# physimals/fabber_core

Hardware: AMD Instinct MI355X
Metric: voxels/sec to VB convergence (higher is better)
Workload: dtype f64; 1 GPU; BASELINE configs[2]: bi-exponential (examples biexp), white noise, 100 timepoints, max-iterations 50; voxels_per_gpu=1000000, total_voxels=1000000, params=4, need_f=False, parallelism=voxel-shard x1, input_dtype=f32, bad_voxels=55

## Files before the change

fabber_core_amd/csrc/vb_lane_kernel.h:

```cpp
#pragma once

#include "vb_math.h"
#include "vb_models.h"

namespace fvb
{
template <int P>
constexpr int lane_waves()
{
#ifdef FVB_LANE_WAVES_PER_SIMD
    return FVB_LANE_WAVES_PER_SIMD;
#else
    return P <= 2 ? 3 : (P >= 7 ? 1 : 2);
#endif
}
template <int P>
constexpr int lane_prefetch_depth()
{
#ifdef FVB_PREFETCH_DEPTH
    return FVB_PREFETCH_DEPTH;
#else
    return P <= 2 ? 2 : 4;
#endif
}
// ... 175 lines not shown
        if constexpr (ACC)
        {
            if (precise)
                sweep.step_acc(ma, t, tp, tp2, tp3, rden, g, J);
            else
                sweep.eval_jac(ma, t, tp, tp2, tp3, rden, g, J);
        }
        else
            sweep.eval_jac(ma, t, tp, tp2, tp3, rden, g, J);
        if (phi_index)
        {
#pragma unroll
            for (int i = 0; i < P; i++)
                bad_jac |= !is_finite(J[i]);
        }
        if (phi_index)
            bad_offset |= !is_finite(g);
        else
            g_total += g;
        const bool unmasked = phi_index ? (phi_index[t] != 255) : true;
        if (unmasked)
        {
            const double r = y_cur - g;
#pragma unroll
            for (int i = 0; i < P; i++)
            {
#pragma unroll
                for (int j = 0; j <= i; j++)
                    mo.A[tri(i, j)] += J[i] * J[j];
                mo.u[i] += J[i] * r;
            }
            mo.s += r * r;
        }
    };
    FVB_FOR_EACH_TIMEPOINT(lane_prefetch_depth<P>(), ka, v, V, T, step)
    if (!phi_index)
    {
        bad_offset = !is_finite(g_total);
#pragma unroll
        for (int i = 0; i < P; i++)
            bad_jac |= !is_finite(mo.A[tri(i, i)]);
    }
    return bad_offset ? FVB_BAD_OFFSET : (bad_jac ? FVB_BAD_JACOBIAN : FVB_OK);
}

enum
{
    FEED_TILES_F32 = 0,
    FEED_TILES_F64 = 1,
    FEED_STRIDED = 2
};

template <int FEED>
struct FeedTraits
{
    typedef float raw;
};
template <>
struct FeedTraits<FEED_TILES_F64>
{
    typedef double raw;
};

template <typename RAW>
struct Tile
{
    static constexpr int G = 16 / (int)sizeof(RAW);
    typedef RAW vec __attribute__((ext_vector_type(16 / sizeof(RAW))));
    static FVB_HD size_t groups(int T)
    {
        return (size_t)((T + G - 1) / G);
    }
    static FVB_HD size_t block_elems(int T)
    {
        return groups(T) * 64 * G;
    }
    static FVB_HD size_t bytes(int V, int T)
    {
        return (size_t)((V + 63) / 64) * block_elems(T) * sizeof(RAW);
    }
};

template <typename RAW>
__global__ __launch_bounds__(256) void retile_series(const RAW *__restrict__ data, RAW *__restrict__ tiles, int V, int T)
{
    typedef Tile<RAW> TL;
    const int v = blockIdx.x * 256 + threadIdx.x;
    if (v >= V)
        return;
    const int n_groups = (int)TL::groups(T);
    typename TL::vec *dst = (typename TL::vec *)(tiles + (size_t)(v >> 6) * TL::block_elems(T)) + (v & 63);
    const RAW *src = data + v;
    for (int g = 0; g < n_groups; g++)
    {
        typename TL::vec q;
#pragma unroll
        for (int j = 0; j < TL::G; j++)
        {
            const int t = g * TL::G + j;
            q[j] = (t < T) ? src[(size_t)t * V] : RAW(0);
        }
        dst[(size_t)g * 64] = q;
    }
}

template <typename RAW, class Body>
__device__ __forceinline__ void for_each_timepoint_tiled(const RAW *lane_tile, int T, Body body)
{
    typedef Tile<RAW> TL;
    constexpr int TRIP = 8;
    constexpr int NL = TRIP / TL::G;
    const int n_trips = T / TRIP;
    if (n_trips > 0)
    {
        const typename TL::vec *p = (const typename TL::vec *)lane_tile;
        typename TL::vec qa[NL], qb[NL];
        auto fetch = [&](typename TL::vec(&q)[NL], int trip) {
#pragma unroll
            for (int l = 0; l < NL; l++)
                q[l] = p[(size_t)(trip * NL + l) * 64];
        };
        auto process = [&](const typename TL::vec(&q)[NL], int t0) {
#pragma unroll
            for (int j = 0; j < TRIP; j++)
                body(t0 + j, (double)q[j / TL::G][j % TL::G]);
        };
        fetch(qa, 0);
        int k = 0;
        for (; k + 2 <= n_trips; k += 2)
        {
            fetch(qb, k + 1);
            process(qa, k * TRIP);
            fetch(qa, (k + 2 < n_trips) ? k + 2 : n_trips - 1);
            process(qb, (k + 1) * TRIP);
        }
        if (k < n_trips)
            process(qa, k * TRIP);
    }
#pragma nounroll
    for (int t = n_trips * TRIP; t < T; t++)
        body(t, (double)lane_tile[(size_t)(t / TL::G) * 64 * TL::G + (t % TL::G)]);
}

template <class Model, int P, typename RAW>
__device__ __forceinline__ int recentre_tiles(const KernelArgs &ka, const ModelArgs &ma, const RAW *lane_tile,
    const double (&centre)[P], Moments<P> &mo, bool precise, double *sweep_park = nullptr)
{
    typedef Tile<RAW> TL;
    constexpr int PT = P * (P + 1) / 2;
    constexpr int TRIP = 8;
    constexpr int NL = TRIP / TL::G;
    static_assert(FVB_EXP_RESYNC == 1 || FVB_EXP_RESYNC == 2 || FVB_EXP_RESYNC == 4 || FVB_EXP_RESYNC == 8,
        "the resync period must divide the trip length");
    const int T = ka.cfg.n_times;
    double tp[P], tp2[P], tp3[P], rden[P];
#pragma unroll
    for (int i = 0; i < P; i++)
    {
        const int tr = ka.cfg.transform[i];
        double delta = centre[i] * 1e-5;
        if (delta < 0)
            delta = -delta;
        if (delta < 1e-10)
            delta = 1e-10;
        const double c2 = centre[i] + delta;
        const double c3 = centre[i] - delta;
        tp[i] = to_model(tr, centre[i]);
        tp2[i] = to_model(tr, c2);
        tp3[i] = to_model(tr, c3);
        rden[i] = 1.0 / (c2 - c3);
        mo.ml[i] = centre[i];
    }
    if (sweep_park)
    {
        double *q = sweep_park + (threadIdx.x & 63);
#pragma unroll
        for (int i = 0; i < P; i++)
        {
            q[(0 * P + i) * 64] = tp[i];
            q[(1 * P + i) * 64] = tp2[i];
            q[(2 * P + i) * 64] = tp3[i];
            q[(3 * P + i) * 64] = rden[i];
        }
    }
#pragma unroll
    for (int i = 0; i < PT; i++)
        mo.A[i] = 0;
#pragma unroll
    for (int i = 0; i < P; i++)
        mo.u[i] = 0;
    mo.s = 0;
    mo.precise = precise;
    typename Model::Sweep sweep;
    sweep.init(ma, tp, tp2, tp3);
    sweep.set_precise(false);
    double g_total = 0;
    auto accumulate = [&](double y_cur, double g, const double(&J)[P]) {
        g_total += g;
        const double r = y_cur - g;
#pragma unroll
        for (int i = 0; i < P; i++)
        {
#pragma unroll
            for (int j = 0; j <= i; j++)
                mo.A[tri(i, j)] += J[i] * J[j];
            mo.u[i] += J[i] * r;
        }
        mo.s += r * r;
    };
    int t = 0;
    const int n_trips = precise ? 0 : T / TRIP;
    if (n_trips > 0)
    {
        const typename TL::vec *p = (const typename TL::vec *)lane_tile;
        typename TL::vec qa[NL], qb[NL];
        auto fetch = [&](typename TL::vec(&q)[NL], int trip) {
#pragma unroll
            for (int l = 0; l < NL; l++)
                q[l] = p[(size_t)(trip * NL + l) * 64];
        };
        auto process = [&](const typename TL::vec(&q)[NL], int t0) {
#pragma unroll
            for (int j = 0; j < TRIP; j++)
            {
                double g, J[P];
                if (j % FVB_EXP_RESYNC == 0)
                    sweep.template step_fast<true>(ma, t0 + j, tp, tp2, tp3, rden, g, J);
                else
                    sweep.template step_fast<false>(ma, t0 + j, tp, tp2, tp3, rden, g, J);
                accumulate((double)q[j / TL::G][j % TL::G], g, J);
            }
        };
        fetch(qa, 0);
        int k = 0;
        for (; k + 2 <= n_trips; k += 2)
        {
            fetch(qb, k + 1);
            process(qa, k * TRIP);
            fetch(qa, (k + 2 < n_trips) ? k + 2 : n_trips - 1);
            process(qb, (k + 1) * TRIP);
        }
        if (k < n_trips)
            process(qa, k * TRIP);
        t = n_trips * TRIP;
    }
#pragma nounroll
    for (; t < T; t++)
    {
        const double y_cur = (double)lane_tile[(size_t)(t / TL::G) * 64 * TL::G + (t % TL::G)];
        double g, J[P];
        sweep.step_any(ma, t, tp, tp2, tp3, rden, g, J, precise);
        accumulate(y_cur, g, J);
    }
    bool bad_jac = false;
#pragma unroll
    for (int i = 0; i < P; i++)
        bad_jac |= !is_finite(mo.A[tri(i, i)]);
    return !is_finite(g_total) ? FVB_BAD_OFFSET : (bad_jac ? FVB_BAD_JACOBIAN : FVB_OK);
}

template <int P, bool NEEDF>
__device__ __forceinline__ bool apply_priors(const KernelArgs &ka, int v, int it, VoxelState<P> &st, double &Fprior)
{
    bool ok = true;
    bool any_ard = false;
#pragma unroll
    for (int k = 0; k < P; k++)
        any_ard |= (ka.cfg.prior_type[k] == FVB_PRIOR_ARD);
    if (any_ard)
        ok = ensure_cov<P>(st);
#pragma unroll
    for (int k = 0; k < P; k++)
    {
        const int type = ka.cfg.prior_type[k];
        double fk = 0;
        double pm_k, pprec_k;
        if (type == FVB_PRIOR_ARD)
        {
            const double post_mean = st.m[k];
            const double post_cov = st.Sig[tri(k, k)];
            const double new_cov = post_mean * post_mean + post_cov;
            pprec_k = 1.0 / ((it == 0) ? ka.cfg.prior_var[k] : new_cov);
            pm_k = ka.cfg.prior_mean[k];
            if (NEEDF)
            {
                const double bb = 2 / new_cov;
                fk = -1.5 * (log(bb) + digamma(0.5)) - 0.5 - gammaln(0.5) - 0.5 * log(bb);
            }
        }
        else if (type == FVB_PRIOR_IMAGE)
        {
            pm_k = ka.cfg.image_prior[k][v];
            pprec_k = ka.cfg.prior_prec[k];
        }
        else
        {
            pm_k = ka.cfg.prior_mean[k];
            pprec_k = ka.cfg.prior_prec[k];
        }
        st.pm[k] = pm_k;
        st.pprec[k] = pprec_k;
        Fprior = fk;
    }
    return ok;
}

template <int P>
__device__ __forceinline__ double theta_rhs_base(double phibar, const Moments<P> &mo, int i)
{
    double aml = 0;
#pragma unroll
    for (int j = 0; j < P; j++)
        aml = __builtin_fma(mo.A[tri(i, j)], mo.ml[j], aml);
    return phibar * (mo.u[i] + aml);
}
__device__ __forceinline__ double theta_rhs(double base, double prior_prec, double prior_mean)
{
    return __builtin_fma(prior_prec, prior_mean, base);
}
template <int P>
__device__ __forceinline__ double theta_mean(const double *Sig, const double (&rhs)[P], int i)
{
    double s = 0;
#pragma unroll
    for (int j = 0; j < P; j++)
        s = __builtin_fma(Sig[tri(i, j)], rhs[j], s);
    return s;
}

template <int P>
__device__ __forceinline__ bool update_theta(VoxelState<P> &st, const Moments<P> &mo, double alpha)
{
    constexpr int PT = P * (P + 1) / 2;
    const double phibar = st.b * st.c;
#pragma unroll
    for (int i = 0; i < P; i++)
#pragma unroll
        for (int j = 0; j <= i; j++)
            st.Lam[tri(i, j)] = phibar * mo.A[tri(i, j)] + ((i == j) ? st.pprec[i] : 0.0);
    st.precValid = true;
    st.covValid = false;
    if (alpha <= 0.0)
    {
        double rhs[P];
#pragma unroll
        for (int i = 0; i < P; i++)
            rhs[i] = theta_rhs(theta_rhs_base<P>(phibar, mo, i), st.pprec[i], st.pm[i]);
        if (!ensure_cov<P>(st))
            return false;
#pragma unroll
        for (int i = 0; i < P; i++)
            st.m[i] = theta_mean<P>(st.Sig, rhs, i);
    }
    else
    {
        double Delta[P], Mx[PT], Mi[PT];
#pragma unroll
        for (int i = 0; i < P; i++)
            Delta[i] = phibar * mo.u[i] + st.pprec[i] * st.pm[i] - st.pprec[i] * mo.ml[i];
#pragma unroll
        for (int i = 0; i < PT; i++)
            Mx[i] = st.Lam[i];
#pragma unroll
        for (int i = 0; i < P; i++)
            Mx[tri(i, i)] += alpha * st.Lam[tri(i, i)];
        double la;
        int sg;
        if (ldl_inverse<P>(Mx, Mi, la, sg))
        {
#pragma unroll
            for (int i = 0; i < P; i++)
            {
                double s = 0;
#pragma unroll
                for (int j = 0; j < P; j++)
                    s += Mi[tri(i, j)] * Delta[j];
                st.m[i] = mo.ml[i] + s;
            }
        }
    }
    return true;
}

template <int P>
__device__ __forceinline__ double trace_SA(const VoxelState<P> &st, const Moments<P> &mo)
{
    double tr = 0;
#pragma unroll
    for (int i = 0; i < P; i++)
#pragma unroll
        for (int j = 0; j < P; j++)
            tr += st.Sig[tri(i, j)] * mo.A[tri(i, j)];
    return tr;
}

template <int P>
__device__ __forceinline__ void residual_terms(
    const VoxelState<P> &st, const Moments<P> &mo, double tol, double &kk, double &trSA, bool &lost)
{
    double d[P];
#pragma unroll
    for (int i = 0; i < P; i++)
        d[i] = st.m[i] - mo.ml[i];
    double du = 0, dAd = 0;
    trSA = 0;
// ... 532 lines not shown
    {
        lg = gammaln(c);
        dg = digamma(c);
    }
    const double noise_terms = free_energy_noise_terms(ka, b, c, lg, dg, fk.prior_const);
    const double prior_logdet = (fk.prior_is_const && priors_applied) ? fk.prior_logdet : prior_log_determinant<P>(st);
    double F = theta_terms + noise_terms + data_terms + prior_logdet;
    finite = is_finite(F);
    return F + Fprior;
}

template <int P>
__device__ __forceinline__ bool free_energy_would_be_finite(const VoxelState<P> &st, double theta_terms, double data_terms)
{
    bool ok = is_finite(theta_terms + data_terms) && st.b > 0 && st.c > 0 && is_finite(st.b * st.c) && is_finite(st.c);
#pragma unroll
    for (int i = 0; i < P; i++)
        ok = ok && is_finite(st.pprec[i]) && st.pprec[i] != 0;
    return ok;
}

template <int P>
__device__ __forceinline__ void save_state(const KernelArgs &ka, int v, const VoxelState<P> &st)
{
    constexpr int PT = P * (P + 1) / 2;
    const size_t V = (size_t)ka.cfg.n_voxels;
    double *p = ka.save + v;
    int r = 0;
#pragma unroll
    for (int i = 0; i < P; i++)
        p[(size_t)(r++) * V] = st.m[i];
#pragma unroll
    for (int i = 0; i < PT; i++)
        p[(size_t)(r++) * V] = st.Lam[i];
#pragma unroll
    for (int i = 0; i < PT; i++)
        p[(size_t)(r++) * V] = st.Sig[i];
#pragma unroll
    for (int i = 0; i < P; i++)
        p[(size_t)(r++) * V] = st.pm[i];
#pragma unroll
    for (int i = 0; i < P; i++)
        p[(size_t)(r++) * V] = st.pprec[i];
    p[(size_t)(r++) * V] = st.b;
    p[(size_t)(r++) * V] = st.c;
    p[(size_t)(r++) * V] = (st.precValid ? 1.0 : 0.0) + (st.covValid ? 2.0 : 0.0) + 4.0 * 0;
}

template <int P>
__device__ __forceinline__ void restore_state(const KernelArgs &ka, int v, VoxelState<P> &st)
{
    constexpr int PT = P * (P + 1) / 2;
    const size_t V = (size_t)ka.cfg.n_voxels;
    const double *p = ka.save + v;
    int r = 0;
#pragma unroll
    for (int i = 0; i < P; i++)
        st.m[i] = p[(size_t)(r++) * V];
#pragma unroll
    for (int i = 0; i < PT; i++)
        st.Lam[i] = p[(size_t)(r++) * V];
#pragma unroll
    for (int i = 0; i < PT; i++)
        st.Sig[i] = p[(size_t)(r++) * V];
#pragma unroll
    for (int i = 0; i < P; i++)
        st.pm[i] = p[(size_t)(r++) * V];
#pragma unroll
    for (int i = 0; i < P; i++)
        st.pprec[i] = p[(size_t)(r++) * V];
    st.b = p[(size_t)(r++) * V];
    st.c = p[(size_t)(r++) * V];
    const int flags = (int)p[(size_t)(r++) * V];
    if (flags & 1)
    {
        st.precValid = true;
        st.covValid = false;
    }
    else
    {
        st.precValid = false;
        st.covValid = true;
    }
}

template <class Model, int P, bool NEEDF, int FEED, bool WATCH = NEEDF>
__global__ __launch_bounds__(64, lane_waves<P>()) void vb_lane_kernel(const KernelArgs ka)
{
    constexpr int PT = P * (P + 1) / 2;
    typedef typename FeedTraits<FEED>::raw RAW;
    const int v_lane = blockIdx.x * 64 + threadIdx.x;
    const int v = (v_lane < ka.cfg.n_voxels) ? v_lane : ka.cfg.n_voxels - 1;
    const int T = ka.cfg.n_times;
    const size_t V = (size_t)ka.cfg.n_voxels;

    ModelArgs ma;
    ma.iopt0 = ka.cfg.model_iopt[0];
    ma.dopt0 = ka.cfg.model_dopt[0];
    ma.design = ka.cfg.design;
    const RAW *wave_tile = (FEED == FEED_STRIDED) ? nullptr : (const RAW *)ka.tiles + (size_t)blockIdx.x * Tile<RAW>::block_elems(T);
    const RAW *lane_tile = (FEED == FEED_STRIDED) ? nullptr : wave_tile + (size_t)(v & 63) * Tile<RAW>::G;

    VoxelState<P> st;
    Moments<P> mo;
    int status = FVB_OK;
    __shared__ double park_lds[ParkPlan<P, NEEDF>::ROWS * 64];
    __shared__ double rescue_row[64];
    constexpr bool SWEEP_PARKED = (FEED != FEED_STRIDED) && SweepPark<P, NEEDF>::FITS;
    __shared__ double sweep_lds[SWEEP_PARKED ? SweepPark<P, NEEDF>::ROWS * 64 : 1];
    double *park = park_lds + threadIdx.x;
    double *sweep_park = SWEEP_PARKED ? sweep_lds : nullptr;

    if (ka.cfg.init_mvn)
    {
        constexpr int n = P + 1;
        constexpr int nCov = n * (n + 1) / 2;
        const double *src = ka.cfg.init_mvn + v;
#pragma unroll
        for (int i = 0; i < PT; i++)
            st.Sig[i] = src[(size_t)i * V];
#pragma unroll
        for (int i = 0; i < P; i++)
            st.m[i] = src[(size_t)(nCov + i) * V];
        const double nm = src[(size_t)(nCov + P) * V];
        const double nv = src[(size_t)tri(P, P) * V];
        st.b = nv / nm;
        st.c = nm / st.b;
    }
    else
    {
#pragma unroll
        for (int i = 0; i < PT; i++)
            st.Sig[i] = 0;
#pragma unroll
        for (int i = 0; i < P; i++)
        {
            st.m[i] = (ka.cfg.prior_type[i] == FVB_PRIOR_IMAGE) ? ka.cfg.image_prior[i][v] : ka.cfg.post_mean[i];
            st.Sig[tri(i, i)] = ka.cfg.post_var[i];
        }
        if (Model::needs_data_max)
        {
            double data_max;
            if (FEED == FEED_STRIDED)
            {
                data_max = load_data(ka, v);
                for (int t = 1; t < T; t++)
                {
                    const double y = load_data(ka, (size_t)t * V + v);
                    data_max = (y > data_max) ? y : data_max;
                }
            }
            else
            {
                constexpr int G = Tile<RAW>::G;
                data_max = (double)lane_tile[0];
#pragma nounroll
                for (int t = 1; t < T; t++)
                {
                    const double y = (double)lane_tile[(size_t)(t / G) * 64 * G + (t % G)];
                    data_max = (y > data_max) ? y : data_max;
                }
            }
            Model::init_posterior(ma, data_max, st.m);
        }
#pragma unroll
        for (int i = 0; i < P; i++)
        {
            const int tr = ka.cfg.transform[i];
            st.m[i] = to_fabber(tr, st.m[i]);
            st.Sig[tri(i, i)] = to_fabber_var(tr, st.Sig[tri(i, i)]);
        }
        st.b = ka.cfg.noise_post_b[0];
        st.c = ka.cfg.noise_post_c[0];
    }
    st.covValid = true;
    st.precValid = false;
    st.logdetLam = 0;
#pragma unroll
    for (int i = 0; i < P; i++)
    {
        st.pm[i] = 0;
        st.pprec[i] = 1;
    }

    double F = 1234.5678;
    double Fprior = 0;
    int it = 0;
    int hist_len = 0;
    bool setup_failed = false;

    ConvState conv;
    conv_init(conv, ka.cfg.convergence, ka.cfg.max_iterations, ka.cfg.max_trials, ka.cfg.min_fchange);
    conv_reset(conv);
    const bool use_save = WATCH && (ka.save != nullptr);
    enum
    {
        FIRST,
        ITERATING,
        REVERTED
    };
    int phase = FIRST;
    int n_lin = 0;
    bool logdet_valid = false;

    enum
    {
        LINEARISE,
        PRIORS,
        THETA,
        NOISE
    };
    int stage = LINEARISE;
    double kk = 0, trSA = 0;
    FreeEnergyConsts<P> fk;
    if (NEEDF)
        fk.init(ka);
    bool pending = false, priors_applied = false;
    double pending_part = 0, pending_b = 0, pending_c = 0;
#define FVB_VOXEL_FAILS(CODE, B, C)                                                                          \
    {                                                                                                        \
        status = (CODE);                                                                                     \
        pending_b = (B);                                                                                     \
        pending_c = (C);                                                                                     \
        break;                                                                                               \
    }
    for (;;)
    {
        bool want_f = NEEDF;
        double f_kk, f_tr;
        double b_before = 0, c_before = 0;
        if (stage == LINEARISE)
        {
            park_state<P, NEEDF>(park, st);
            if (FEED == FEED_STRIDED)
                status = recentre<Model, P>(ka, ma, v, st.m, mo, n_lin < ka.precise_passes);
            else
                status = recentre_tiles<Model, P, RAW>(ka, ma, lane_tile, st.m, mo, n_lin < ka.precise_passes, sweep_park);
            n_lin = (phase == REVERTED) ? n_lin : n_lin + 1;
            unpark_state<P, NEEDF>(park, st);
            if (status != FVB_OK)
            {
                setup_failed = (phase == FIRST);
                FVB_VOXEL_FAILS(status, st.b, st.c)
            }
            if (phase == FIRST)
            {
                if (use_save)
                    save_posterior<P>(ka, v, st, logdet_valid);
                want_f = false;
            }
        }
        else if (stage == PRIORS)
        {
            if (use_save && conv_need_save(conv))
                save_posterior<P>(ka, v, st, logdet_valid);
            if (!apply_priors<P, NEEDF>(ka, v, it, st, Fprior))
                FVB_VOXEL_FAILS(FVB_BAD_RESULT, st.b, st.c)
            priors_applied = true;
        }
        else if (stage == THETA)
        {
            if (!update_theta<P>(st, mo, WATCH ? conv_lm_alpha(conv) : 0.0) || !ensure_cov<P>(st))
                FVB_VOXEL_FAILS(FVB_BAD_RESULT, st.b, st.c)
            st.precValid = false;
            logdet_valid = true;
            if (FEED == FEED_STRIDED)
                residual_and_trace<Model, P, NEEDF>(ka, ma, v, st, mo, kk, trSA, park, rescue_row);
            else
                residual_and_trace_adaptive<Model, P, NEEDF, RAW, SWEEP_PARKED>(ka, ma, v, st, mo, kk, trSA, park, rescue_row, wave_tile, sweep_park);
        }
        else
        {
            b_before = st.b;
            c_before = st.c;
            update_noise<P>(ka, st, kk, trSA);
        }
        if (want_f)
        {
            if (stage == LINEARISE || stage == PRIORS)
            {
                if (!ensure_cov<P>(st))
                    FVB_VOXEL_FAILS(FVB_BAD_RESULT, st.b, st.c)
                f_kk = mo.s;
                f_tr = trace_SA<P>(st, mo);
            }
            else
            {
                f_kk = kk;
                f_tr = trSA;
            }
            double theta_terms, data_terms;
            if (!free_energy_partial<P>(ka, st, f_kk, f_tr, logdet_valid, theta_terms, data_terms))
                FVB_VOXEL_FAILS(FVB_BAD_RESULT, st.b, st.c)
            if (stage == LINEARISE)
            {
                bool fin = true;
                const double Fn = free_energy_full<P>(ka, fk, st, st.b, st.c, priors_applied && phase != REVERTED, theta_terms, data_terms, Fprior, fin);
                if (!fin)
                    FVB_VOXEL_FAILS(FVB_BAD_FREE_ENERGY, st.b, st.c)
                F = Fn;
                pending = false;
            }
            else
            {
                if (!free_energy_would_be_finite<P>(st, theta_terms, data_terms))
                {
                    const bool noise_stage = (stage == NOISE);
                    FVB_VOXEL_FAILS(FVB_BAD_FREE_ENERGY, noise_stage ? b_before : st.b, noise_stage ? c_before : st.c)
                }
                pending_part = theta_terms + data_terms;
                pending = true;
            }
        }
// ... 76 lines not shown
```

fabber_core_amd/csrc/vb_models.h:

```cpp
#pragma once

#include "vb_math.h"

#ifdef FVB_STRICT_MODELS
#define FVB_MODEL_FP _Pragma("clang fp contract(off)")
#else
#define FVB_MODEL_FP _Pragma("clang fp contract(fast)")
#endif

namespace fvb
{
struct ModelArgs
{
    int32_t iopt0;
    double dopt0;
    const double *design;
    const double *lin;
    int32_t lin_T;
    const double *exp_table;
    const double *consts;
    int32_t n_consts;
    int32_t model;
};

template <class Model, int P>
struct PointwiseSweep
{
    FVB_HD void init(const ModelArgs &, const double (&)[P], const double (&)[P], const double (&)[P])
    {
    }
    FVB_HD void set_precise(bool)
    {
    }
    FVB_HD void eval(const ModelArgs &ma, int t, const double (&tp)[P], const double (&tp2)[P], const double (&tp3)[P],
        double &g, double (&f2)[P], double (&f3)[P])
    {
        FVB_MODEL_FP
        g = Model::eval(ma, t, tp);
#pragma unroll
        for (int i = 0; i < P; i++)
        {
            double q[P];
#pragma unroll
            for (int j = 0; j < P; j++)
                q[j] = tp[j];
            q[i] = tp2[i];
            f2[i] = Model::eval(ma, t, q);
            q[i] = tp3[i];
            f3[i] = Model::eval(ma, t, q);
        }
    }
    FVB_HD void eval_jac(const ModelArgs &ma, int t, const double (&tp)[P], const double (&tp2)[P], const double (&tp3)[P],
        const double (&rden)[P], double &g, double (&J)[P])
    {
        FVB_MODEL_FP
        double f2[P], f3[P];
        eval(ma, t, tp, tp2, tp3, g, f2, f3);
#pragma unroll
        for (int i = 0; i < P; i++)
            J[i] = (f2[i] - f3[i]) * rden[i];
    }
    template <bool EXACT>
    FVB_HD void step_fast(const ModelArgs &ma, int t, const double (&tp)[P], const double (&tp2)[P],
        const double (&tp3)[P], const double (&rden)[P], double &g, double (&J)[P])
    {
        eval_jac(ma, t, tp, tp2, tp3, rden, g, J);
    }
    FVB_HD void step_any(const ModelArgs &ma, int t, const double (&tp)[P], const double (&tp2)[P],
        const double (&tp3)[P], const double (&rden)[P], double &g, double (&J)[P], bool)
    {
        eval_jac(ma, t, tp, tp2, tp3, rden, g, J);
    }
};

template <class Model, int P>
struct LinearInParameterSweep
{
    double d2[P], d3[P];
    bool precise;
    FVB_HD void init(const ModelArgs &, const double (&tp)[P], const double (&tp2)[P], const double (&tp3)[P])
    {
        precise = false;
#pragma unroll
        for (int i = 0; i < P; i++)
        {
            d2[i] = tp2[i] - tp[i];
            d3[i] = tp3[i] - tp[i];
        }
    }
    FVB_HD void set_precise(bool p)
    {
        precise = p;
    }
    FVB_HD void eval(const ModelArgs &ma, int t, const double (&tp)[P], const double (&tp2)[P], const double (&tp3)[P],
        double &g, double (&f2)[P], double (&f3)[P])
    {
        FVB_MODEL_FP
        if (precise)
        {
            PointwiseSweep<Model, P> pw;
            pw.eval(ma, t, tp, tp2, tp3, g, f2, f3);
            return;
        }
        g = Model::eval(ma, t, tp);
#pragma unroll
        for (int i = 0; i < P; i++)
        {
            const double b = Model::basis(ma, t, i);
            f2[i] = g + b * d2[i];
            f3[i] = g + b * d3[i];
        }
    }
    FVB_HD void eval_jac(const ModelArgs &ma, int t, const double (&tp)[P], const double (&tp2)[P], const double (&tp3)[P],
        const double (&rden)[P], double &g, double (&J)[P])
    {
        FVB_MODEL_FP
        if (precise)
        {
            PointwiseSweep<Model, P> pw;
            pw.eval_jac(ma, t, tp, tp2, tp3, rden, g, J);
            return;
        }
        g = Model::eval(ma, t, tp);
#pragma unroll
        for (int i = 0; i < P; i++)
            J[i] = Model::basis(ma, t, i) * ((tp2[i] - tp3[i]) * rden[i]);
    }
    template <bool EXACT>
    FVB_HD void step_fast(const ModelArgs &ma, int t, const double (&tp)[P], const double (&tp2)[P],
        const double (&tp3)[P], const double (&rden)[P], double &g, double (&J)[P])
    {
        FVB_MODEL_FP
        g = Model::eval(ma, t, tp);
#pragma unroll
        for (int i = 0; i < P; i++)
            J[i] = Model::basis(ma, t, i) * ((tp2[i] - tp3[i]) * rden[i]);
    }
    FVB_HD void step_any(const ModelArgs &ma, int t, const double (&tp)[P], const double (&tp2)[P],
        const double (&tp3)[P], const double (&rden)[P], double &g, double (&J)[P], bool prec)
    {
        precise = prec;
        eval_jac(ma, t, tp, tp2, tp3, rden, g, J);
    }
};

template <int P>
struct PolyModel
{
    static constexpr bool host_evaluated = false;
    static constexpr int model_id = FVB_MODEL_POLY;
    typedef LinearInParameterSweep<PolyModel<P>, P> Sweep;
    static FVB_HD double basis(const ModelArgs &, int t, int n)
    {
        int pw = 1;
        for (int k = 0; k < n; k++)
            pw *= t + 1;
        return (double)pw;
    }
    static FVB_HD double eval(const ModelArgs &, int t, const double (&p)[P])
    {
        FVB_MODEL_FP
        const int i = t + 1;
        double res = 0;
        int pw = 1;
#pragma unroll
        for (int n = 0; n < P; n++)
        {
            res += p[n] * pw;
            pw *= i;
        }
        return res;
    }
    static FVB_HD void init_posterior(const ModelArgs &, double, double (&)[P])
    {
    }
    static constexpr bool needs_data_max = false;
};

template <int P>
struct LinearModel
{
    static constexpr bool host_evaluated = false;
    static constexpr int model_id = FVB_MODEL_LINEAR;
    typedef LinearInParameterSweep<LinearModel<P>, P> Sweep;
    static FVB_HD double basis(const ModelArgs &a, int t, int n)
    {
        return a.design[(size_t)t * P + n];
    }
    static FVB_HD double eval(const ModelArgs &a, int t, const double (&p)[P])
    {
        FVB_MODEL_FP
        const double *row = a.design + (size_t)t * P;
        double s = 0;
#pragma unroll
        for (int j = 0; j < P; j++)
            s += row[j] * (p[j] - 0.0);
        return s + 0.0;
    }
    static FVB_HD void init_posterior(const ModelArgs &, double, double (&)[P])
    {
    }
    static constexpr bool needs_data_max = false;
};

template <int P>
struct ExpModel
{
    static constexpr bool host_evaluated = false;
    static_assert(P % 2 == 0, "exp model has 2 parameters per exponential");
    static constexpr int model_id = FVB_MODEL_EXP;
    static FVB_HD double eval(const ModelArgs &a, int t, const double (&p)[P])
    {
        FVB_MODEL_FP
        const double tt = double(t) * a.dopt0;
        double res = 0;
#pragma unroll
        for (int i = 0; i < P / 2; i++)
        {
            double val = p[2 * i] * exp(-p[2 * i + 1] * tt);
            res += val;
        }
        return res;
    }
    static FVB_HD void init_posterior(const ModelArgs &, double data_max, double (&means)[P])
    {
#pragma unroll
        for (int i = 0; i < P / 2; i++)
            means[2 * i] = data_max / (P / 2 + i);
    }
    static constexpr bool needs_data_max = true;

#ifndef FVB_EXP_RESYNC
#define FVB_EXP_RESYNC 8
#endif
    struct Sweep
    {
        static constexpr int N = P / 2;
        double e0[N], e2[N], e3[N], s0[N], s2[N], s3[N];
        bool precise;
        FVB_HD void init(const ModelArgs &a, const double (&tp)[P], const double (&tp2)[P], const double (&tp3)[P])
        {
            FVB_MODEL_FP
            precise = false;
            if (FVB_EXP_RESYNC > 1)
            {
#pragma unroll
                for (int i = 0; i < N; i++)
                {
                    s0[i] = exp(-tp[2 * i + 1] * a.dopt0);
                    s2[i] = exp(-tp2[2 * i + 1] * a.dopt0);
                    s3[i] = exp(-tp3[2 * i + 1] * a.dopt0);
                }
            }
        }
        FVB_HD void set_precise(bool p)
        {
            precise = p;
        }
        FVB_HD void advance(const ModelArgs &a, int t, const double (&tp)[P], const double (&tp2)[P], const double (&tp3)[P])
        {
            FVB_MODEL_FP
            if (FVB_EXP_RESYNC <= 1 || precise || (t % FVB_EXP_RESYNC) == 0)
            {
                const double tt = double(t) * a.dopt0;
#pragma unroll
                for (int i = 0; i < N; i++)
                {
                    e0[i] = exp(-tp[2 * i + 1] * tt);
                    e2[i] = exp(-tp2[2 * i + 1] * tt);
                    e3[i] = exp(-tp3[2 * i + 1] * tt);
                }
            }
            else
            {
#pragma unroll
                for (int i = 0; i < N; i++)
                {
                    e0[i] *= s0[i];
                    e2[i] *= s2[i];
                    e3[i] *= s3[i];
                }
            }
        }
        FVB_HD void eval(const ModelArgs &a, int t, const double (&tp)[P], const double (&tp2)[P], const double (&tp3)[P],
            double &g, double (&f2)[P], double (&f3)[P])
        {
            FVB_MODEL_FP
            advance(a, t, tp, tp2, tp3);
            combine(tp, tp2, tp3, g, f2, f3);
        }
        FVB_HD void resync(const ModelArgs &a, int t, const double (&tp)[P], const double (&tp2)[P], const double (&tp3)[P])
        {
            FVB_MODEL_FP
            const double tt = double(t) * a.dopt0;
#pragma unroll
            for (int i = 0; i < N; i++)
            {
                e0[i] = exp(-tp[2 * i + 1] * tt);
                e2[i] = exp(-tp2[2 * i + 1] * tt);
                e3[i] = exp(-tp3[2 * i + 1] * tt);
            }
        }
        FVB_HD void resync_acc(const ModelArgs &a, int t, const double (&tp)[P], const double (&tp2)[P], const double (&tp3)[P])
        {
            FVB_MODEL_FP
            const double tt = double(t) * a.dopt0;
#pragma unroll
            for (int i = 0; i < N; i++)
            {
                e0[i] = exp_acc(-tp[2 * i + 1] * tt, a.exp_table);
                e2[i] = exp_acc(-tp2[2 * i + 1] * tt, a.exp_table);
                e3[i] = exp_acc(-tp3[2 * i + 1] * tt, a.exp_table);
            }
        }
        FVB_HD void multiply()
        {
            FVB_MODEL_FP
#pragma unroll
            for (int i = 0; i < N; i++)
            {
                e0[i] *= s0[i];
                e2[i] *= s2[i];
                e3[i] *= s3[i];
            }
        }
        FVB_HD void combine(const double (&tp)[P], const double (&tp2)[P], const double (&tp3)[P], double &g,
            double (&f2)[P], double (&f3)[P])
        {
            FVB_MODEL_FP
            double val[N];
#pragma unroll
            for (int j = 0; j < N; j++)
                val[j] = tp[2 * j] * e0[j];
            double res = val[0];
#pragma unroll
            for (int j = 1; j < N; j++)
                res += val[j];
            g = res;
#pragma unroll
            for (int i = 0; i < N; i++)
            {
                double a2 = (i == 0) ? tp2[0] * e0[0] : val[0];
                double a3 = (i == 0) ? tp3[0] * e0[0] : val[0];
                double r2 = (i == 0) ? tp[0] * e2[0] : val[0];
                double r3 = (i == 0) ? tp[0] * e3[0] : val[0];
#pragma unroll
                for (int j = 1; j < N; j++)
                {
                    a2 += (j == i) ? tp2[2 * i] * e0[i] : val[j];
                    a3 += (j == i) ? tp3[2 * i] * e0[i] : val[j];
                    r2 += (j == i) ? tp[2 * i] * e2[i] : val[j];
                    r3 += (j == i) ? tp[2 * i] * e3[i] : val[j];
                }
                f2[2 * i] = a2;
                f3[2 * i] = a3;
                f2[2 * i + 1] = r2;
                f3[2 * i + 1] = r3;
            }
        }
        FVB_HD void eval_jac(const ModelArgs &a, int t, const double (&tp)[P], const double (&tp2)[P], const double (&tp3)[P],
            const double (&rden)[P], double &g, double (&J)[P])
        {
            FVB_MODEL_FP
            double f2[P], f3[P];
            eval(a, t, tp, tp2, tp3, g, f2, f3);
#pragma unroll
            for (int i = 0; i < P; i++)
                J[i] = (f2[i] - f3[i]) * rden[i];
        }
        template <bool EXACT>
        FVB_HD void step_fast(const ModelArgs &a, int t, const double (&tp)[P], const double (&tp2)[P],
            const double (&tp3)[P], const double (&rden)[P], double &g, double (&J)[P])
        {
            FVB_MODEL_FP
            if (EXACT || FVB_EXP_RESYNC <= 1)
                resync(a, t, tp, tp2, tp3);
            else
                multiply();
            double f2[P], f3[P];
            combine(tp, tp2, tp3, g, f2, f3);
#pragma unroll
            for (int i = 0; i < P; i++)
                J[i] = (f2[i] - f3[i]) * rden[i];
        }
        FVB_HD void step_acc(const ModelArgs &a, int t, const double (&tp)[P], const double (&tp2)[P], const double (&tp3)[P],
            const double (&rden)[P], double &g, double (&J)[P])
        {
            FVB_MODEL_FP
            resync_acc(a, t, tp, tp2, tp3);
            double f2[P], f3[P];
            combine(tp, tp2, tp3, g, f2, f3);
#pragma unroll
            for (int i = 0; i < P; i++)
                J[i] = (f2[i] - f3[i]) * rden[i];
        }
        FVB_HD void step_any(const ModelArgs &a, int t, const double (&tp)[P], const double (&tp2)[P],
            const double (&tp3)[P], const double (&rden)[P], double &g, double (&J)[P], bool prec)
        {
            FVB_MODEL_FP
            if (FVB_EXP_RESYNC <= 1 || prec || (t % FVB_EXP_RESYNC) == 0)
                resync(a, t, tp, tp2, tp3);
            else
                multiply();
            double f2[P], f3[P];
            combine(tp, tp2, tp3, g, f2, f3);
#pragma unroll
            for (int i = 0; i < P; i++)
                J[i] = (f2[i] - f3[i]) * rden[i];
        }
    };
};

template <int P>
struct HostLinModel
{
    static constexpr bool host_evaluated = true;
    static constexpr int model_id = FVB_MODEL_HOSTJAC;
    static constexpr bool needs_data_max = false;
    static FVB_HD void init_posterior(const ModelArgs &, double, double (&)[P])
    {
    }
    static FVB_HD double eval(const ModelArgs &, int, const double (&)[P])
    {
        return __builtin_nan("");
    }
    struct Sweep
    {
        const double *g_row, *j_rows;
        FVB_HD void init(const ModelArgs &a, const double (&)[P], const double (&)[P], const double (&)[P])
        {
            g_row = a.lin;
            j_rows = a.lin + a.lin_T;
        }
        FVB_HD void set_precise(bool)
        {
        }
        FVB_HD void eval_jac(const ModelArgs &, int t, const double (&)[P], const double (&)[P], const double (&)[P],
            const double (&)[P], double &g, double (&J)[P])
        {
            g = g_row[t];
#pragma unroll
            for (int i = 0; i < P; i++)
                J[i] = j_rows[(size_t)t * P + i];
        }
    };
};

FVB_HD double eval_model_runtime(int model, const ModelArgs &a, int P, int t, const double *p)
{
    FVB_MODEL_FP
    switch (model)
    {
    case FVB_MODEL_POLY:
    {
        const int i = t + 1;
        double res = 0;
        int pw = 1;
        for (int n = 0; n < P; n++)
        {
            res += p[n] * pw;
            pw *= i;
        }
        return res;
    }
    case FVB_MODEL_LINEAR:
    {
        const double *row = a.design + (size_t)t * P;
        double s = 0;
        for (int j = 0; j < P; j++)
            s += row[j] * (p[j] - 0.0);
        return s + 0.0;
    }
    case FVB_MODEL_EXP:
    {
        const double tt = double(t) * a.dopt0;
        double res = 0;
        for (int i = 0; i < P / 2; i++)
            res += p[2 * i] * exp(-p[2 * i + 1] * tt);
        return res;
    }
    default:
        return NAN;
    }
}

}
```

Measured before the change: 74.65 million voxels/s.

## Run precise and remainder sweeps by prefetched trips and vectorise data-max scan

Restructures recentre_tiles so the tile prefetch is hoisted before the setup math. Precise sweeps and the tail remainder for multi-exponential models now go through the trip-based prefetched loop instead of a scalar per-timepoint loop. Adds an FMA-fused sum variant in combine for two-component models, and rewrites the data_max initial scan to use vector tile loads with a lookahead buffer. This aims to hide load latency and cut per-element index arithmetic, at the cost of more code paths and slightly different floating-point rounding from the fused sums.

```diff
diff --git a/fabber_core_amd/csrc/vb_lane_kernel.h b/fabber_core_amd/csrc/vb_lane_kernel.h
--- a/fabber_core_amd/csrc/vb_lane_kernel.h
+++ b/fabber_core_amd/csrc/vb_lane_kernel.h
@@ -351,7 +351,23 @@
     constexpr int NL = TRIP / TL::G;
     static_assert(FVB_EXP_RESYNC == 1 || FVB_EXP_RESYNC == 2 || FVB_EXP_RESYNC == 4 || FVB_EXP_RESYNC == 8,
         "the resync period must divide the trip length");
+    typedef typename Model::Sweep Sweep;
+    constexpr bool BY_TRIPS = Sweep::pointwise_by_trips;
     const int T = ka.cfg.n_times;
+    const int n_trips = (!BY_TRIPS && precise) ? 0 : T / TRIP;
+    const int rem = T - n_trips * TRIP;
+    const int last_group = (int)TL::groups(T) - 1;
+    const typename TL::vec *p = (const typename TL::vec *)lane_tile;
+    typename TL::vec qa[NL], qb[NL];
+    auto fetch = [&](typename TL::vec(&q)[NL], int trip) {
+#pragma unroll
+        for (int l = 0; l < NL; l++)
+        {
+            const int g = trip * NL + l;
+            q[l] = p[(size_t)(g < last_group ? g : last_group) * 64];
+        }
+    };
+    fetch(qa, 0);
     double tp[P], tp2[P], tp3[P], rden[P];
 #pragma unroll
     for (int i = 0; i < P; i++)
@@ -390,7 +406,7 @@
         mo.u[i] = 0;
     mo.s = 0;
     mo.precise = precise;
-    typename Model::Sweep sweep;
+    Sweep sweep;
     sweep.init(ma, tp, tp2, tp3);
     sweep.set_precise(false);
     double g_total = 0;
@@ -407,49 +423,128 @@
         }
         mo.s += r * r;
     };
-    int t = 0;
-    const int n_trips = precise ? 0 : T / TRIP;
-    if (n_trips > 0)
-    {
-        const typename TL::vec *p = (const typename TL::vec *)lane_tile;
-        typename TL::vec qa[NL], qb[NL];
-        auto fetch = [&](typename TL::vec(&q)[NL], int trip) {
-#pragma unroll
-            for (int l = 0; l < NL; l++)
-                q[l] = p[(size_t)(trip * NL + l) * 64];
-        };
-        auto process = [&](const typename TL::vec(&q)[NL], int t0) {
-#pragma unroll
-            for (int j = 0; j < TRIP; j++)
-            {
-                double g, J[P];
-                if (j % FVB_EXP_RESYNC == 0)
-                    sweep.template step_fast<true>(ma, t0 + j, tp, tp2, tp3, rden, g, J);
+    auto step = [&](bool exact, bool pointwise, bool fuse_last, int t, double &g, double(&J)[P]) {
+        if constexpr (Sweep::states_fusion)
+        {
+            if (pointwise)
+            {
+                if (fuse_last)
+                    sweep.template step_pointwise<2>(ma, t, tp, tp2, tp3, rden, g, J);
                 else
-                    sweep.template step_fast<false>(ma, t0 + j, tp, tp2, tp3, rden, g, J);
-                accumulate((double)q[j / TL::G][j % TL::G], g, J);
-            }
-        };
-        fetch(qa, 0);
+                    sweep.template step_pointwise<1>(ma, t, tp, tp2, tp3, rden, g, J);
+            }
+            else if (exact)
+            {
+                if (fuse_last)
+                    sweep.template step_fast<true, 2>(ma, t, tp, tp2, tp3, rden, g, J);
+                else
+                    sweep.template step_fast<true, 1>(ma, t, tp, tp2, tp3, rden, g, J);
+            }
+            else
+            {
+                if (fuse_last)
+                    sweep.template step_fast<false, 2>(ma, t, tp, tp2, tp3, rden, g, J);
+                else
+                    sweep.template step_fast<false, 1>(ma, t, tp, tp2, tp3, rden, g, J);
+            }
+        }
+        else
+        {
+            if (pointwise)
+                sweep.step_pointwise(ma, t, tp, tp2, tp3, rden, g, J);
+            else if (exact)
+                sweep.template step_fast<true>(ma, t, tp, tp2, tp3, rden, g, J);
+            else
+                sweep.template step_fast<false>(ma, t, tp, tp2, tp3, rden, g, J);
+        }
+    };
+    auto process = [&](const typename TL::vec(&q)[NL], int t0, bool second_of_pair) {
+#pragma unroll
+        for (int j = 0; j < TRIP; j++)
+        {
+            double g, J[P];
+            step(j % FVB_EXP_RESYNC == 0, false, j >= TRIP - (second_of_pair ? 2 : 1), t0 + j, g, J);
+            accumulate((double)q[j / TL::G][j % TL::G], g, J);
+        }
+    };
+    auto process_pointwise = [&](const typename TL::vec(&q)[NL], int t0) {
+#pragma unroll
+        for (int j = 0; j < TRIP; j++)
+        {
+            double g, J[P];
+            step(true, true, true, t0 + j, g, J);
+            accumulate((double)q[j / TL::G][j % TL::G], g, J);
+        }
+    };
+    auto next_set = [&]() {
+#pragma unroll
+        for (int l = 0; l < NL; l++)
+            qa[l] = qb[l];
+    };
+    if (precise)
+    {
+#pragma nounroll
+        for (int k = 0; k < n_trips; k++)
+        {
+            fetch(qb, k + 1);
+            process_pointwise(qa, k * TRIP);
+            next_set();
+        }
+    }
+    else
+    {
         int k = 0;
         for (; k + 2 <= n_trips; k += 2)
         {
             fetch(qb, k + 1);
-            process(qa, k * TRIP);
-            fetch(qa, (k + 2 < n_trips) ? k + 2 : n_trips - 1);
-            process(qb, (k + 1) * TRIP);
+            process(qa, k * TRIP, false);
+            fetch(qa, k + 2);
+            process(qb, (k + 1) * TRIP, true);
         }
         if (k < n_trips)
-            process(qa, k * TRIP);
-        t = n_trips * TRIP;
-    }
+        {
+            fetch(qb, k + 1);
+            process(qa, k * TRIP, false);
+            next_set();
+        }
+    }
+    int t_rem = n_trips * TRIP;
+    if constexpr (!BY_TRIPS)
+    {
 #pragma nounroll
-    for (; t < T; t++)
-    {
-        const double y_cur = (double)lane_tile[(size_t)(t / TL::G) * 64 * TL::G + (t % TL::G)];
-        double g, J[P];
-        sweep.step_any(ma, t, tp, tp2, tp3, rden, g, J, precise);
-        accumulate(y_cur, g, J);
+        for (int t = t_rem; t < T; t++)
+        {
+            const double y_cur = (double)lane_tile[(size_t)(t / TL::G) * 64 * TL::G + (t % TL::G)];
+            double g, J[P];
+            sweep.step_any(ma, t, tp, tp2, tp3, rden, g, J, precise);
+            accumulate(y_cur, g, J);
+        }
+    }
+    if constexpr (BY_TRIPS)
+        asm volatile("" : "+s"(t_rem));
+#pragma unroll
+    for (int j = 0; j < TRIP - 1; j++)
+    {
+        if (BY_TRIPS && j < rem)
+        {
+            const int t = t_rem + j;
+            double g, J[P];
+            if (j % FVB_EXP_RESYNC == 0)
+            {
+                if (Sweep::exact_is_pointwise || !precise)
+                    step(true, false, true, t, g, J);
+                else
+                    step(true, true, true, t, g, J);
+            }
+            else
+            {
+                if (precise)
+                    step(false, true, true, t, g, J);
+                else
+                    step(false, false, true, t, g, J);
+            }
+            accumulate((double)qa[j / TL::G][j % TL::G], g, J);
+        }
     }
     bool bad_jac = false;
 #pragma unroll
@@ -1288,13 +1383,34 @@
             }
             else
             {
-                constexpr int G = Tile<RAW>::G;
-                data_max = (double)lane_tile[0];
-#pragma nounroll
-                for (int t = 1; t < T; t++)
+                typedef Tile<RAW> TL;
+                constexpr int NB = 8;
+                const typename TL::vec *p = (const typename TL::vec *)lane_tile;
+                const int n_groups = (int)TL::groups(T);
+                typename TL::vec q[NB];
+#pragma unroll
+                for (int l = 0; l < NB; l++)
+                    q[l] = p[(size_t)(l < n_groups ? l : n_groups - 1) * 64];
+                data_max = (double)q[0][0];
+                for (int g0 = 0; g0 < n_groups; g0 += NB)
                 {
-                    const double y = (double)lane_tile[(size_t)(t / G) * 64 * G + (t % G)];
-                    data_max = (y > data_max) ? y : data_max;
+                    typename TL::vec qc[NB];
+#pragma unroll
+                    for (int l = 0; l < NB; l++)
+                    {
+                        qc[l] = q[l];
+                        const int g = g0 + NB + l;
+                        q[l] = p[(size_t)(g < n_groups ? g : n_groups - 1) * 64];
+                    }
+#pragma unroll
+                    for (int l = 0; l < NB; l++)
+#pragma unroll
+                        for (int j = 0; j < TL::G; j++)
+                            if ((g0 + l) * TL::G + j < T)
+                            {
+                                const double y = (double)qc[l][j];
+                                data_max = (y > data_max) ? y : data_max;
+                            }
                 }
             }
             Model::init_posterior(ma, data_max, st.m);
diff --git a/fabber_core_amd/csrc/vb_models.h b/fabber_core_amd/csrc/vb_models.h
--- a/fabber_core_amd/csrc/vb_models.h
+++ b/fabber_core_amd/csrc/vb_models.h
@@ -71,6 +71,14 @@
     {
         eval_jac(ma, t, tp, tp2, tp3, rden, g, J);
     }
+    static constexpr bool exact_is_pointwise = true;
+    static constexpr bool states_fusion = false;
+    static constexpr bool pointwise_by_trips = false;
+    FVB_HD void step_pointwise(const ModelArgs &ma, int t, const double (&tp)[P], const double (&tp2)[P],
+        const double (&tp3)[P], const double (&rden)[P], double &g, double (&J)[P])
+    {
+        eval_jac(ma, t, tp, tp2, tp3, rden, g, J);
+    }
 };
 
 template <class Model, int P>
@@ -141,6 +149,16 @@
     {
         precise = prec;
         eval_jac(ma, t, tp, tp2, tp3, rden, g, J);
+    }
+    static constexpr bool exact_is_pointwise = false;
+    static constexpr bool states_fusion = false;
+    static constexpr bool pointwise_by_trips = false;
+    FVB_HD void step_pointwise(const ModelArgs &ma, int t, const double (&tp)[P], const double (&tp2)[P],
+        const double (&tp3)[P], const double (&rden)[P], double &g, double (&J)[P])
+    {
+        FVB_MODEL_FP
+        PointwiseSweep<Model, P> pw;
+        pw.eval_jac(ma, t, tp, tp2, tp3, rden, g, J);
     }
 };
 
@@ -324,6 +342,7 @@
                 e3[i] *= s3[i];
             }
         }
+        template <int FUSE = 0>
         FVB_HD void combine(const double (&tp)[P], const double (&tp2)[P], const double (&tp3)[P], double &g,
             double (&f2)[P], double (&f3)[P])
         {
@@ -332,10 +351,18 @@
 #pragma unroll
             for (int j = 0; j < N; j++)
                 val[j] = tp[2 * j] * e0[j];
-            double res = val[0];
-#pragma unroll
-            for (int j = 1; j < N; j++)
-                res += val[j];
+            double res;
+            if (N == 2 && FUSE == 1)
+                res = __builtin_fma(tp[0], e0[0], val[1]);
+            else if (N == 2 && FUSE == 2)
+                res = __builtin_fma(tp[2], e0[N - 1], val[0]);
+            else
+            {
+                res = val[0];
+#pragma unroll
+                for (int j = 1; j < N; j++)
+                    res += val[j];
+            }
             g = res;
 #pragma unroll
             for (int i = 0; i < N; i++)
@@ -368,7 +395,9 @@
             for (int i = 0; i < P; i++)
                 J[i] = (f2[i] - f3[i]) * rden[i];
         }
-        template <bool EXACT>
+        static constexpr bool states_fusion = true;
+        static constexpr bool pointwise_by_trips = true;
+        template <bool EXACT, int FUSE = 0>
         FVB_HD void step_fast(const ModelArgs &a, int t, const double (&tp)[P], const double (&tp2)[P],
             const double (&tp3)[P], const double (&rden)[P], double &g, double (&J)[P])
         {
@@ -378,7 +407,7 @@
             else
                 multiply();
             double f2[P], f3[P];
-            combine(tp, tp2, tp3, g, f2, f3);
+            combine<FUSE>(tp, tp2, tp3, g, f2, f3);
 #pragma unroll
             for (int i = 0; i < P; i++)
                 J[i] = (f2[i] - f3[i]) * rden[i];
@@ -408,6 +437,13 @@
             for (int i = 0; i < P; i++)
                 J[i] = (f2[i] - f3[i]) * rden[i];
         }
+        static constexpr bool exact_is_pointwise = true;
+        template <int FUSE = 0>
+        FVB_HD void step_pointwise(const ModelArgs &a, int t, const double (&tp)[P], const double (&tp2)[P],
+            const double (&tp3)[P], const double (&rden)[P], double &g, double (&J)[P])
+        {
+            step_fast<true, FUSE>(a, t, tp, tp2, tp3, rden, g, J);
+        }
     };
 };
 
```

Result: faster. 75.52 million voxels/s (median of 6 runs) (+1.2%).
